# AE-HYU/monte_carlo_localization

Hardware: AMD Instinct MI355X
Metric: MCL updates/sec (particle*beam/s) (higher is better)
Workload: dtype f64; 1 GPU; 4194304 particles/GPU x 1081 beams, Spielberg_map (2000x2000 @ 0.05796), initial cloud N((0.0, 0.0, 0.0),(0.5 m,0.5 m,0.4 rad)) (tracking regime), action (0.05, 0.0, 0.01), stock sensor/motion params, multinomial resampling, Philox seed 42; the timed updates follow 5 warm-up updates (the particle set has resampled to motion-noise width); particles_total=4194304, beams=1081, parallelism=single GPU

## Files before the change

include/mcl_hip_engine.h:

```cpp
#ifndef MCL_HIP_ENGINE_H
#define MCL_HIP_ENGINE_H

#include <stddef.h>
#include <stdint.h>

#ifdef __cplusplus
extern "C" {
#endif

#define MCL_ABI_VERSION 1

typedef struct mcl_engine mcl_engine_t;

typedef enum {
    MCL_OK = 0,
    MCL_ERR_INVALID_ARG = -1,
    MCL_ERR_NOT_READY = -2,
    MCL_ERR_HIP = -3,
    MCL_ERR_NO_DEVICE = -4,
    MCL_ERR_UNSUPPORTED = -5,
    MCL_ERR_PEER = -6,
    MCL_ERR_TIMEOUT = -7
} mcl_status;

// ... 48 lines not shown

int mcl_set_map(mcl_engine_t *h, const int8_t *data, uint32_t width, uint32_t height,
                float resolution, double origin_x, double origin_y);
int mcl_get_max_range_px(const mcl_engine_t *h, int32_t *out);
int mcl_get_sensor_table(const mcl_engine_t *h, double *out, size_t n);

int mcl_set_beam_angles(mcl_engine_t *h, const float *angles, int32_t n_beams);

int mcl_set_particles(mcl_engine_t *h, const double *xyz_colmajor, const double *weights, int64_t n);
int mcl_set_particles_shard(mcl_engine_t *h, const double *xyz_colmajor, const double *weights, int64_t n, double max_weight_of_the_whole_set);
int mcl_init_particles_pose(mcl_engine_t *h, const double pose[3], int64_t n, int64_t first_global_index, int64_t n_total);
int mcl_init_global(mcl_engine_t *h, int64_t n, int64_t first_global_index, int64_t n_total);
int mcl_get_particles(mcl_engine_t *h, double *xyz_colmajor, int64_t n);
int mcl_get_weights(mcl_engine_t *h, double *weights, int64_t n);
int mcl_sample_particles(mcl_engine_t *h, int32_t k, const double *uniforms, double *out_colmajor);
int mcl_particle_mean(mcl_engine_t *h, double out[3]);

int mcl_update(mcl_engine_t *h, const double action[3], const float *obs, int32_t n_beams,
               const double *normals_nx3, const double *uniforms_n);
int mcl_update_scan(mcl_engine_t *h, const double action[3], const float *ranges, int32_t n_ranges, int32_t angle_step);
int mcl_sensor_update(mcl_engine_t *h, const float *obs, int32_t n_beams);

int mcl_expected_pose(mcl_engine_t *h, double out[3]);

int mcl_get_stage_timings(const mcl_engine_t *h, double ms[6]);

int mcl_get_resample_indices(mcl_engine_t *h, int32_t *idx, int64_t n);
int mcl_get_ray_steps(mcl_engine_t *h, uint8_t *steps, size_t n);
int mcl_get_ray_steps16(mcl_engine_t *h, uint16_t *steps, size_t n);
int mcl_get_log_weights(mcl_engine_t *h, double *logw, int64_t n);
int mcl_get_counters(mcl_engine_t *h, uint64_t out[4]);
int mcl_get_compact_list(const mcl_engine_t *h, int64_t *n_entries, int32_t *used_by_last_update);
int mcl_set_debug_count_probes(mcl_engine_t *h, int32_t on);
int mcl_get_ray_kernel_ms(const mcl_engine_t *h, double *ms);
int mcl_get_ray_kernel_id(const mcl_engine_t *h, int32_t *kernel);
int mcl_get_ray_kernel_variant(const mcl_engine_t *h, int32_t out[3]);
int mcl_get_planned_ray_kernel(const mcl_engine_t *h, int64_t n_particles, int32_t *kernel, const char **reason);
int mcl_get_effective_sample_size(const mcl_engine_t *h, double *n_eff, int32_t *resampled_last_update);

typedef struct {
    int64_t min_particles, max_particles;
    double err;
    double z;
    double bin_x_m, bin_y_m;
    int32_t n_theta_bins;
    int32_t round_to;
    int32_t shrink_permille;
    int32_t reserved;
} mcl_kld_config_t;
void mcl_default_kld_config(mcl_kld_config_t *k);
int mcl_set_kld(mcl_engine_t *h, const mcl_kld_config_t *k);
int mcl_get_particle_count(const mcl_engine_t *h, int64_t *n);
int mcl_get_kld_state(const mcl_engine_t *h, int64_t *bins_last, int64_t *n_next);
int mcl_host_kld_bins(const double *x, const double *y, const double *th, int64_t n, uint32_t width, uint32_t height,
                      float resolution, double origin_x, double origin_y, const mcl_kld_config_t *k, int64_t *bins);
int mcl_host_kld_target(const mcl_kld_config_t *k, int64_t bins, int64_t n_current, int64_t *n_next);

typedef struct {
    double bin_x_m, bin_y_m;
    int32_t n_theta_bins;
    int32_t reserved;
} mcl_cluster_config_t;
typedef struct {
    uint64_t weight_q;
    double weight;
    int64_t n_particles, n_bins, first_bin;
// ... 299 lines not shown
```

monte_carlo_localization_amd/csrc/mcl_engine.hip:

```cpp
#include "../../include/mcl_hip_engine.h"

#include <hip/hip_runtime.h>
#include <hip/hip_ext.h>
#include <rocprim/device/device_radix_sort.hpp>

#include <algorithm>
#include <chrono>
#include <cmath>
#include <cstdio>
#include <cstring>
#include <string>
#include <vector>

#include "mcl_engine_internal.h"
#include "mcl_kernels.h"
#include "mcl_host_math.h"
#include "mcl_lfield.h"

static_assert(MCL_WEDGES == mcl::kWedges || MCL_KWEDGES != 16, "include/mcl_hip_engine.h and csrc/mcl_wedge.h disagree");

using namespace mcl_host;

namespace {

// ... 159 lines not shown
void launch_layout(mcl_engine *h, hipStream_t stream, int64_t n, int *bbox, int *tilemark, int *tilemap)
{
    const auto [ntx_abs, nty_abs, tiles_ok] = sort_tiles(h);
    const int bstride = n >= (1 << 20) ? 16 : 1;
    hipLaunchKernelGGL(mcl::k_cell_bbox, dim3((unsigned)std::min<int64_t>((n / bstride + 255) / 256, 128)), dim3(256), 0, stream, h->d_pc, n,
                       bstride, h->Wp, h->Hp, bbox, tiles_ok ? tilemark : (int *)nullptr, ntx_abs);
    if (tiles_ok) hipLaunchKernelGGL(mcl::k_tile_compact, dim3(1), dim3(1024), 0, stream, bbox, tilemark, tilemap, ntx_abs * nty_abs);
}

int launch_far_windowed(mcl_engine *h, const mcl::RayArgs &a, int64_t n, bool count)
{
    const unsigned nb = (unsigned)((n + mcl::kFarTile - 1) / mcl::kFarTile);
    const uint32_t *flags32 = reinterpret_cast<const uint32_t *>(h->d_far.p);
    hipLaunchKernelGGL(mcl::k_far_count, dim3(nb), dim3(256), 0, h->stream, flags32, n, a.far_count, h->d_far_cnt);
    hipLaunchKernelGGL(mcl::k_far_spine, dim3(1), dim3(1024), 0, h->stream, h->d_far_cnt, (int)nb, a.far_count);
    hipLaunchKernelGGL(mcl::k_far_scatter, dim3(nb), dim3(256), 0, h->stream, flags32, n, a.far_count, h->d_far_cnt, h->d_far_sorted);
    const size_t lds = (size_t)h->tw_cells * h->tw_cells / 2;
    if (count) hipLaunchKernelGGL((mcl::k_rays_skip<1, true, true>), dim3(h->num_cu), dim3(mcl::kRayThreads), lds, h->stream, a);
    else hipLaunchKernelGGL((mcl::k_rays_skip<1, false, true>), dim3(h->num_cu), dim3(mcl::kRayThreads), lds, h->stream, a);
    HIPCHK(h, hipGetLastError());
    return MCL_OK;
}

struct RayPlan {
    int mode = 0;
    bool lists = false, ordered = false, sweep = false;
    bool count = false;
    bool timed = false;
    int R = 1;
    int grid = 1;
    size_t lds = 0;
    int nsl = 1, items_per_slice = 4, sweep_g = 1;
    int nseg = 1, fix_split = 1;
    unsigned long long segcap = 0;
    unsigned gfar = 1;
    bool hyb = false, glob = false, rec = false, pairs = false;
    size_t qlds = 0;
    bool far_windowed = false, radix = false;
    bool constants_ready = false, stale_layout = false, keys_written = false, clear_folded = false, obs_wait = false;
    bool heading_form = false;
    mcl::PrepClear clear_passed{};
};

void plan_work_lists(const mcl_engine *h, int64_t n, RayPlan &p)
{
    const int spc = h->env.qslices_per_cu > 0 ? h->env.qslices_per_cu : 32;
    p.nsl = (int)std::max<int64_t>(1, std::min<int64_t>((int64_t)spc * h->num_cu, (n + 255) / 256));
    if (p.ordered) {
        int64_t slice_len = h->env.cell_slice > 0 ? std::max<int64_t>(64, h->env.cell_slice) : (n >= (1 << 21) ? 4096 : 2048);
        p.nsl = (int)std::max<int64_t>(1, (n + slice_len - 1) / slice_len);
    }
    if (p.sweep) {
        p.sweep_g = h->env.sweep_g > 0 ? h->env.sweep_g : 1;
        if (p.sweep_g > mcl::kWedges || (mcl::kWedges % p.sweep_g) != 0) p.sweep_g = 1;
        p.nsl = (int)((n + mcl::kSwUnit - 1) / mcl::kSwUnit);
    }
    p.items_per_slice = p.sweep ? mcl::kWedges / p.sweep_g : (p.ordered ? mcl::kWedges : 4);
    const int max_wg = 2 * (h->num_cu - h->reserved_cus);
    p.nseg = (int)std::min<int64_t>(max_wg, p.items_per_slice * (int64_t)p.nsl);
    const unsigned long long rays_per_seg = (unsigned long long)n * h->B / p.nseg + 64, seg_div = 256;
    p.segcap = std::max<unsigned long long>(2048, (rays_per_seg / seg_div + 7) & ~7ull);
    unsigned long long share = 2;
    if (p.sweep && h->B > 0) {
        const unsigned long long rays = std::max<unsigned long long>(1, (unsigned long long)n * h->B);
        const unsigned long long by_scan = ((unsigned long long)h->wedge_beams_max * p.items_per_slice + h->B - 1) / h->B;
        share = std::max<unsigned long long>(2, std::min<unsigned long long>(by_scan, (8ull << 20) / rays));
    }
    if ((unsigned long long)n * h->B <= (4ull << 20)) p.segcap = (share * rays_per_seg + 7) & ~7ull;
    p.gfar = (unsigned)std::max<int64_t>(1, std::min<int64_t>(4 * (int64_t)h->num_cu, (n + 15) / 16));
    p.fix_split = std::max(1, std::min(16, (8 * h->num_cu) / std::max(p.nseg, 1)));
}

void plan_sweep_form(mcl_engine *h, RayPlan &p)
{
    p.hyb = sweep_hybrid_decide(h);
    p.glob = h->sweep_global && !p.hyb;
    p.rec = h->rec_ok && h->sweep_rec_layout_ok && h->d_beam_err != nullptr && (size_t)mcl::kSwWinBytes + (size_t)h->ltd_cols * 8 <= 80 * 1024 - 64;
    p.far_windowed = sweep_far_expected(h);
    p.pairs = p.rec && !p.hyb && (h->env.sweep_pairs >= 0 ? h->env.sweep_pairs != 0 : (p.glob || p.far_windowed));
    p.qlds = (p.glob ? 0 : (size_t)mcl::kSwWinBytes) + (p.rec ? (size_t)h->ltd_cols * 8 : 0);
}

RayPlan plan_rays(mcl_engine *h, int64_t n, bool force_skip, bool direct_table)
{
    RayPlan p;
    p.mode = choose_ray_mode(h, n, force_skip);
    p.lists = mode_work_lists(p.mode); p.ordered = mode_orders(p.mode); p.sweep = mode_sweep(p.mode);
    p.count = h->cfg.debug_count_probes != 0;
    p.R = h->cfg.rays_per_lane > 0 ? h->cfg.rays_per_lane : 1;
    p.grid = (int)std::max<int64_t>(1, std::min<int64_t>(h->num_cu, (n + 15) / 16));
    p.lds = (size_t)h->tw_cells * h->tw_cells / 2;
    p.timed = !p.lists && !h->capturing && !direct_table;
    const RayHandoff &ho = h->handoff;
    p.constants_ready = ho.constants;
    p.heading_form = ho.heading && ho.keys && ho.stale_layout && mode_sweep(p.mode) && sort_radix(h, n);
    if (ho.heading && !p.heading_form) p.constants_ready = false;
    if (!p.lists) return p;
    plan_work_lists(h, n, p);
    if (p.sweep) plan_sweep_form(h, p);
    else p.qlds = (size_t)h->qside * h->qside;
    p.stale_layout = p.ordered && ho.stale_layout;
    p.keys_written = ho.keys; p.clear_folded = ho.folded; p.clear_passed = ho.passed; p.obs_wait = ho.obs_wait;
    p.radix = p.ordered && sort_radix(h, n);
// ... 154 lines not shown
    a.sweep_g = p.sweep_g; a.Ltd = h->d_Ltd; a.ltd_cols = h->ltd_cols;
    a.split16 = h->env.sw_split16 >= 0 ? h->env.sw_split16 : 0;
    a.beam_csx = h->sweep_global ? h->d_beam_csxg : h->d_beam_csx; a.beam_pad = h->beam_pad; a.beam_margin = h->beam_margin;
    a.beam_csi = h->d_beam_csi; a.beam_err = h->d_beam_err; a.rec_k = 2.0 * h->rec_c;
    a.distg = h->d_distg; a.distg_stride = h->distg_stride; a.distg_pitch = h->distg_pitch;
    a.items = h->d_items; a.centres = h->d_centres; a.nitems = 0; a.nitems_ptr = h->d_nitems; a.unit_sums = h->d_unit_sums; a.unit_begin = h->d_unit_begin; a.slot_space = 1;
    MCL_TRY(h->d_far_list.reserve(h, (size_t)h->cap));
    MCL_TRY(h->d_far_sorted.reserve(h, (size_t)h->cap));
    MCL_TRY(h->d_far_cnt.reserve(h, (size_t)h->cap / mcl::kFarTile + 2));
    a.far_sorted = h->d_far_sorted;
    a.far_windowed = p.far_windowed ? 1 : 0;
    a.far_list = h->d_far_list; a.far_count = h->d_result + 15;
    return MCL_OK;
}

template <bool COUNT>
int ray_kernel_lists(mcl_engine *h, const RayPlan &p, const mcl::RayArgs &a)
{
    const dim3 qg((unsigned)p.nseg), b(mcl::kRayThreads);
    if (!p.sweep) HIPCHK(h, hipEventRecord(h->ev[EV_K0], h->stream));
    if (p.hyb) hipExtLaunchKernelGGL((mcl::k_rays_sweep<COUNT, false, true, false, true>), qg, b, p.qlds, h->stream, nullptr, h->ev[EV_K1], 0, a);
    else if (p.glob && p.rec) hipExtLaunchKernelGGL((mcl::k_rays_sweep<COUNT, true, true, true>), qg, b, p.qlds, h->stream, nullptr, h->ev[EV_K1], 0, a);
    else if (p.glob) hipExtLaunchKernelGGL((mcl::k_rays_sweep<COUNT, true>), qg, b, p.qlds, h->stream, nullptr, h->ev[EV_K1], 0, a);
    else if (p.sweep && p.rec && p.pairs) hipExtLaunchKernelGGL((mcl::k_rays_sweep<COUNT, false, true, true>), qg, b, p.qlds, h->stream, nullptr, h->ev[EV_K1], 0, a);
    else if (p.sweep && p.rec) hipExtLaunchKernelGGL((mcl::k_rays_sweep<COUNT, false, true>), qg, b, p.qlds, h->stream, nullptr, h->ev[EV_K1], 0, a);
    else if (p.sweep) hipExtLaunchKernelGGL((mcl::k_rays_sweep<COUNT>), qg, b, p.qlds, h->stream, nullptr, h->ev[EV_K1], 0, a);
#ifdef MCL_LEGACY_RAY_KERNELS
    else if (p.ordered) hipLaunchKernelGGL((mcl::k_rays_cell<COUNT>), qg, b, p.qlds, h->stream, a);
    else hipLaunchKernelGGL((mcl::k_rays_quad<COUNT>), qg, b, p.qlds, h->stream, a);
#endif
    if (!p.sweep) HIPCHK(h, hipEventRecord(h->ev[EV_K1], h->stream));
    if (p.sweep && p.far_windowed) MCL_TRY(launch_far_windowed(h, a, a.n, COUNT));
    hipLaunchKernelGGL((mcl::k_rays_far<COUNT>), dim3(p.gfar), b, 0, h->stream, a);
    hipLaunchKernelGGL((mcl::k_rays_fix<COUNT>), dim3(p.nseg * p.fix_split), dim3(256), 0, h->stream, a);
    hipLaunchKernelGGL((mcl::k_rays_exact<COUNT>), dim3(2 * h->num_cu), dim3(256), 0, h->stream, a);
    return MCL_OK;
}
template int ray_kernel_lists<true>(mcl_engine *, const RayPlan &, const mcl::RayArgs &);
template int ray_kernel_lists<false>(mcl_engine *, const RayPlan &, const mcl::RayArgs &);

int ray_kernel(mcl_engine *h, const RayPlan &p, const mcl::RayArgs &a)
{
    if (p.lists) return p.count ? ray_kernel_lists<true>(h, p, a) : ray_kernel_lists<false>(h, p, a);
    const dim3 g(p.grid), b(mcl::kRayThreads);
    if (p.timed) HIPCHK(h, hipEventRecord(h->ev[EV_K0], h->stream));
    if (p.mode == MCL_RAYS_MARCH) ray_kernel_march(h, p, a);
    else if (p.count) hipLaunchKernelGGL((mcl::k_rays_skip<1, true>), g, b, p.lds, h->stream, a);
    else {
        switch (p.R) {
        case 1: hipLaunchKernelGGL((mcl::k_rays_skip<1, false>), g, b, p.lds, h->stream, a); break;
        case 2: hipLaunchKernelGGL((mcl::k_rays_skip<2, false>), g, b, p.lds, h->stream, a); break;
        case 3: hipLaunchKernelGGL((mcl::k_rays_skip<3, false>), g, b, p.lds, h->stream, a); break;
        default: hipLaunchKernelGGL((mcl::k_rays_skip<4, false>), g, b, p.lds, h->stream, a); break;
        }
    }
    if (p.timed) HIPCHK(h, hipEventRecord(h->ev[EV_K1], h->stream));
    return MCL_OK;
}

void ray_combine(mcl_engine *h, const RayPlan &p, int64_t n)
{
    if (p.sweep) {
        hipExtLaunchKernelGGL(mcl::k_combine_logw, dim3(mcl::kRedBlocks), dim3(256), 0, h->stream, nullptr, h->ev[EV_RAYS], 0, n, h->d_perm.p, h->d_logw_acc.p,
                              h->d_logw.p, h->d_maxpart.p, h->d_fix_count.p, p.nseg, p.segcap, h->d_fix_over);
        h->stage_ev.rays_bound = true;
        h->max_partials_ready = true;
    } else {
// ... 363 lines not shown
    h->h_fix_count = h->h_result[12];
    uint64_t qt;
    std::memcpy(&qt, &h->h_scalars[2], 8);
    h->q_total = qt;
    h->global_sums[0] = h->h_scalars[1];
    h->global_sums[1] = h->h_scalars[3];
    h->global_sums[2] = h->h_scalars[4];
    h->global_sums[3] = h->h_scalars[5];
    h->global_sums[4] = h->h_scalars[6];
    if (h->compact_pending) {
        const unsigned long long na = h->h_result[16];
        h->compact_n = na <= (unsigned long long)h->compact_cap ? (int64_t)na : -1;
        h->compact_pending = false;
    }
}

int mcl_abi_version(void) { return MCL_ABI_VERSION; }

const char *mcl_last_error(const mcl_engine_t *h) { return h ? h->err.c_str() : g_create_error.c_str(); }

static EnvKnobs read_knobs()
{
    EnvKnobs k;
    if (const char *e = getenv("MCL_CELL_MIN")) k.cell_min = atoll(e);
    if (const char *e = getenv("MCL_CELL_SLICE")) k.cell_slice = atoll(e);
    if (const char *e = getenv("MCL_QSLICES_PER_CU")) k.qslices_per_cu = atoi(e);
    if (const char *e = getenv("MCL_QSIDE")) k.qside = atoi(e);
    if (const char *e = getenv("MCL_SWEEP_G")) k.sweep_g = atoi(e);
    if (const char *e = getenv("MCL_TINY_POLL")) k.tiny_poll = atoi(e);
    if (const char *e = getenv("MCL_NO_COMPACT")) k.no_compact = atoi(e);
    if (const char *e = getenv("MCL_SORT")) k.sort_radix = std::strcmp(e, "radix") == 0 ? 1 : (std::strcmp(e, "hist") == 0 ? 0 : -1);
    if (const char *e = getenv("MCL_SORT_FINE")) k.sort_fine = atoi(e);
    if (const char *e = getenv("MCL_SORT_FINE_SUB")) k.sort_fine_sub = atoi(e);
    if (const char *e = getenv("MCL_DEBUG_WG")) k.debug_wg = e;
    k.no_bucket_cuts = getenv("MCL_NO_BUCKET_CUTS") != nullptr;
    if (const char *e = getenv("MCL_SWEEP_GLOBAL")) k.sweep_global = atoi(e) != 0;
    if (const char *e = getenv("MCL_SWEEP_HYBRID")) k.sweep_hybrid = atoi(e);
    if (const char *e = getenv("MCL_SW_GUIDE")) k.sw_guide = atoi(e);
    if (const char *e = getenv("MCL_SW_SPLIT16")) k.sw_split16 = atoi(e) != 0;
    if (const char *e = getenv("MCL_SWEEP_PAIRS")) k.sweep_pairs = atoi(e) != 0 ? 1 : 0;
    k.no_obs_overlap = getenv("MCL_NO_OBS_OVERLAP") != nullptr;
    k.no_prep_fold = getenv("MCL_NO_PREP_FOLD") != nullptr;
    k.no_stale_layout = getenv("MCL_NO_STALE_LAYOUT") != nullptr;
    k.comm_no_pregather = getenv("MCL_COMM_NO_PREGATHER") != nullptr;
    k.comm_no_lists = getenv("MCL_COMM_NO_LISTS") != nullptr;
    return k;
}

int mcl_create(const mcl_config_t *cfg, mcl_engine_t **out)
{
    if (cfg && (cfg->resample_neff_permille < 0 || cfg->resample_neff_permille > 1000)) return MCL_ERR_INVALID_ARG;
    g_create_error.clear();
    if (!cfg || !out) { g_create_error = "null argument"; return MCL_ERR_INVALID_ARG; }
    *out = nullptr;
    if (cfg->max_particles <= 0 || cfg->max_particles >= MCL_MAX_TOTAL_PARTICLES || cfg->squash_factor <= 0 || cfg->max_range_m <= 0) {
        g_create_error = "bad config (max_particles must be in [1, 2^27) / squash_factor / max_range_m)";
        return MCL_ERR_INVALID_ARG;
    }
    if (!std::isfinite(cfg->squash_factor) || !std::isfinite(cfg->max_range_m)) {
        g_create_error = "bad config (squash_factor and max_range_m must be finite)";
        return MCL_ERR_INVALID_ARG;
    }
    if (const char *why = bad_sensor_fields(*cfg)) { g_create_error = why; return MCL_ERR_INVALID_ARG; }
    {
        const double disp[3] = {cfg->motion_dispersion_x, cfg->motion_dispersion_y, cfg->motion_dispersion_theta};
        for (double v : disp)
// ... 1079 lines not shown
{
    if (!h || !logw) return MCL_ERR_INVALID_ARG;
    if (!h->have_logw) return MCL_ERR_NOT_READY;
    if (n != h->N) return MCL_ERR_INVALID_ARG;
    HIPCHK(h, hipSetDevice(h->cfg.device));
    HIPCHK(h, hipMemcpyAsync(logw, h->d_logw, (size_t)n * 8, hipMemcpyDeviceToHost, h->stream));
    HIPCHK(h, hipStreamSynchronize(h->stream));
    return MCL_OK;
}

int mcl_get_counters(mcl_engine_t *h, uint64_t out[4])
{
    if (!h || !out) return MCL_ERR_INVALID_ARG;
    for (int i = 0; i < 4; ++i) out[i] = h->h_counters[i];
    return MCL_OK;
}

int mcl_get_compact_list(const mcl_engine_t *h, int64_t *n_entries, int32_t *used_by_last_update)
{
    if (!h || !n_entries || !used_by_last_update) return MCL_ERR_INVALID_ARG;
    *n_entries = h->compact_n;
    *used_by_last_update = h->compact_used ? 1 : 0;
    return MCL_OK;
}

int mcl_set_debug_count_probes(mcl_engine_t *h, int32_t on)
{
    if (!h) return MCL_ERR_INVALID_ARG;
    graph_reset(h);
    h->cfg.debug_count_probes = on ? 1 : 0;
    return MCL_OK;
}

int mcl_get_ray_kernel_ms(const mcl_engine_t *h, double *ms)
{
    if (!h || !ms) return MCL_ERR_INVALID_ARG;
    *ms = h->ray_ms;
    return MCL_OK;
}

int mcl_get_ray_kernel_id(const mcl_engine_t *h, int32_t *kernel)
{
    if (!h || !kernel) return MCL_ERR_INVALID_ARG;
    if (const int rc = lf_refuse_rays(h)) return rc;
    *kernel = h->last_mode;
    return MCL_OK;
}

int mcl_get_ray_kernel_variant(const mcl_engine_t *h, int32_t out[3])
{
    if (!h || !out) return MCL_ERR_INVALID_ARG;
    if (const int rc = lf_refuse_rays(h)) return rc;
    out[0] = h->last_sweep_global; out[1] = h->last_sweep_rec; out[2] = h->last_sweep_pairs;
    return MCL_OK;
}

int mcl_get_planned_ray_kernel(const mcl_engine_t *h, int64_t n_particles, int32_t *kernel, const char **reason)
{
    if (!h || !kernel) return MCL_ERR_INVALID_ARG;
    if (!h->have_map || h->B <= 0) return MCL_ERR_NOT_READY;
    const int64_t n = n_particles > 0 ? n_particles : (h->have_particles ? h->N : h->cap);
    const char *why = "";
    *kernel = choose_ray_mode(h, n, false, &why);
    if (reason) *reason = why ? why : "";
    return MCL_OK;
}
// ... 928 lines not shown
```

monte_carlo_localization_amd/csrc/mcl_engine_internal.h:

```cpp
#pragma once
#include "../../include/mcl_hip_engine.h"

#include <hip/hip_runtime.h>
#include <hip/hip_ext.h>

#include <cstdint>
#include <string>
#include <vector>

#include "mcl_types.h"
#include "mcl_host_math.h"
#include "mcl_buffers.h"

enum { EV_START = 0, EV_RESAMPLE, EV_QUERY, EV_RAYS, EV_SENSOR, EV_K0, EV_K1, EV_COUNT };


constexpr unsigned long long kExactCap = 1ull << 16;
constexpr int kResultWords = 18;
constexpr int kResultStage = 40;
constexpr int kResultStamp = 32;

struct mcl_comm;
void comm_free(struct mcl_comm *c);
void comm_forget(struct mcl_comm *c);
struct mcl_cluster;
void cluster_free(struct mcl_cluster *c);
struct mcl_query;
void query_free(struct mcl_query *q);
struct mcl_search;
void search_free(struct mcl_search *s);
struct mcl_refine;
void refine_free(struct mcl_refine *r);

struct RayHandoff {
    bool constants = false;
    bool stale_layout = false;
    bool keys = false;
    bool heading = false;
    bool folded = false; mcl::PrepClear passed{};
    bool obs_wait = false;
};
struct StageEvents {
    bool rays_bound = false;
    bool query_skipped = false;
};
struct NextLayout {
    bool wanted = false, pending = false, valid = false; int64_t n = 0;
    hipEvent_t ev_children = nullptr, ev_layout = nullptr;
    DevBuf<int> d_bbox_nx, d_tilemap_nx, d_tilemark_nx;
};
struct EnvKnobs {
    int64_t cell_min = 0, cell_slice = 0;
    int qslices_per_cu = 0, qside = 0, sweep_g = 0;
    int tiny_poll = 1, no_compact = 0;
    int sort_radix = -1;
    int sort_fine = -1;
    int sort_fine_sub = -1;
    std::string debug_wg;
    bool no_bucket_cuts = false;
    bool sweep_global = false;
    int sweep_hybrid = 1;
    int sw_guide = 0;
    int sw_split16 = -1;
    int sweep_pairs = -1;
    bool no_obs_overlap = false;
    bool no_prep_fold = false;
    bool no_stale_layout = false;
    bool comm_no_pregather = false;
    bool comm_no_lists = false;
};

struct OrderLast { const int *bbox = nullptr, *tilemap = nullptr; int64_t n = 0; int fine = 0; bool heading = false; };

struct mcl_engine {
    mcl_config_t cfg{};
    int num_cu = 256;
    hipStream_t stream = nullptr;
    hipStream_t stream2 = nullptr;
    std::string err;
    bool have_map = false;
    int W = 0, H = 0, P = 0, Wp = 0, Hp = 0, Wps = 0, tw_cells = 0;
    double res = 0, ox = 0, oy = 0;
    std::vector<double> table;
    DevBuf<int8_t> d_grid;
    DevBuf<uint8_t> d_dist;
    DevBuf<uint8_t> d_dist4;
    DevBuf<uint8_t> d_distq[4];
    DevBuf<uint8_t> d_distw;
    DevBuf<float> d_L;
    DevBuf<double> d_table;
// ... 240 lines not shown
```

monte_carlo_localization_amd/csrc/mcl_kernels.h:

```cpp
#pragma once
#include "mcl_types.h"
#include <type_traits>
#include "mcl_ray_core.h"
#include "mcl_device_math.h"
#include "mcl_wedge.h"
#include "mcl_motion.h"
#include "mcl_sort_key.h"

namespace mcl {

constexpr int kRedBlocks = 1024;
constexpr int kRedThreads = 256;
__device__ __forceinline__ void final_sums_of(const double *__restrict__ part, int nb, double *__restrict__ scalars, double (*sm)[7]);


__device__ __forceinline__ uint64_t wave_incl_scan_u64(uint64_t v, int lane)
{
#pragma unroll
    for (int o = 1; o < 64; o <<= 1) {
        uint64_t t = (uint64_t)__shfl_up((long long)v, o, 64);
        if (lane >= o) v += t;
    }
    return v;
}
// ... 1378 lines not shown
        sy = sm[0][1] + sm[1][1] + sm[2][1] + sm[3][1];
        cnt = sm[0][2] + sm[1][2] + sm[2][2] + sm[3][2];
        out[blockIdx.x] = cnt > 0.0 ? make_double2(sx / cnt, sy / cnt) : make_double2(0.0, 0.0);
    }
}

template <bool GRID = false>
__device__ __forceinline__ int first_beam_in_wedge(double th, const float *__restrict__ angle, int B, int m, double a0, double inv_inc)
{
    int lo = 0, hi = B;
    const double x = ((double)m * (6.283185307179586476925286766559 / kWedges) - th - a0) * inv_inc;
    if (x > -4.0 && x < (double)B + 4.0) {
        const int jg = min(max((int)ceil(x), 0), B);
        if (GRID && fabs(x - rint(x)) > 4e-6 * inv_inc + 1e-6) return jg;
        const bool below = jg == 0 || beam_wedge(th, angle[jg - 1]) < m;
        const bool at = jg == B || beam_wedge(th, angle[jg]) >= m;
        if (below && at) return jg;
        const int l = max(jg - 2, 0), h = min(jg + 2, B);
        if ((l == 0 || beam_wedge(th, angle[l - 1]) < m) && (h == B || beam_wedge(th, angle[h]) >= m)) { lo = l; hi = h; }
    }
    while (lo < hi) {
        const int mid = (lo + hi) >> 1;
        if (beam_wedge(th, angle[mid]) >= m) hi = mid; else lo = mid + 1;
    }
    return lo;
}

#ifdef MCL_LEGACY_RAY_KERNELS
}
#include "mcl_rays_legacy.h"
namespace mcl {
#endif

template <bool COUNT>
__global__ __launch_bounds__(256) void k_rays_fix(RayArgs a)
{
    unsigned long long cnt_exact = 0, cnt_probe = 0, cnt_l2 = 0;
    const int split = max(1, (int)gridDim.x / a.fix_segments);
    const int part = blockIdx.x % split;
    for (int seg = blockIdx.x / split; seg < a.fix_segments; seg += gridDim.x / split) {
    unsigned long long n = 0;
    if (threadIdx.x == 0) n = a.slot_space ? a.fix_count[(size_t)seg * 8] : atomicAdd(&a.fix_count[(size_t)seg * 8], 0ull);
    n = __shfl((long long)n, 0, 64);
    {
        __shared__ unsigned long long n_sh;
        if (threadIdx.x == 0) n_sh = n;
        __syncthreads();
        n = n_sh;
        __syncthreads();
    }
    if (n > a.fix_cap) n = 0;
    cnt_l2 += (threadIdx.x == 0 && part == 0) ? n : 0;
    const unsigned long long *list = a.fix_list + (size_t)seg * a.fix_cap;
    for (unsigned long long k = (unsigned long long)part * blockDim.x + threadIdx.x; k < n; k += (unsigned long long)blockDim.x * split) {
        const unsigned long long e = a.slot_space ? list[k] : atomicAdd(const_cast<unsigned long long *>(&list[k]), 0ull);
        const int64_t p = (int64_t)(e >> 16);
        const int j = (int)(e & 0xFFFF);
        const double4 pci = a.slot_space ? a.pcs[p] : a.pc[p];
        const uint8_t *wfield = nullptr;
        if (a.slot_space && a.distw) {
            const double hth = a.ths[p];
            if (hth == hth && fabs(hth) < 1e6) wfield = a.distw + (size_t)(beam_wedge(hth, a.beam_angle[j]) & (kWedges - 1)) * a.distw_stride;
        }
        const double2 cs = a.beam_cs[j];
        const double ux = pci.x * cs.x - pci.y * cs.y, uy = pci.y * cs.x + pci.x * cs.y;
        const RayOrigin o = ray_origin(a, pci.z, pci.w);
        int r = a.P;
        uint32_t amb = o.amb0;
        unsigned np = 0;
        if (o.sane)
            r = trace_fp64<false, COUNT>(a, nullptr, 0, kOriginBase, o.p0x, o.p0y, ux, uy, first_skip(a, o, wfield ? wfield : a.dist, wfield != nullptr),
                                         amb, np, wfield, wfield != nullptr);
        if (takes_literal_march(a, o.sane, amb)) {
            if (a.exact_list) {
                const unsigned long long slot = atomicAdd(a.exact_count, 1ull);
                if (slot < a.exact_cap) { atomicExch(&a.exact_list[slot], e); continue; }
            }
            const int64_t i = a.slot_space ? (int64_t)a.perm[p] : p;
            r = march_exact(a, a.x[i], a.y[i], a.th[i] + (double)a.beam_angle[j]);
            ++cnt_exact;
        }
        atomicAdd(&a.logw[p], (double)a.Lt[(size_t)r * a.bpad + j]);
        if (a.steps || a.steps16) store_step(a, a.slot_space ? (int64_t)a.perm[p] : p, j, r);
        if (COUNT) cnt_probe += np;
    }
    }
    if (a.counters) {
        if (cnt_exact) atomicAdd(&a.counters[0], cnt_exact);
        if (COUNT && cnt_probe) atomicAdd(&a.counters[2], cnt_probe);
        if (cnt_l2) atomicAdd(&a.counters[3], cnt_l2);
    }
}

template <bool COUNT>
__global__ __launch_bounds__(256) void k_rays_exact(RayArgs a)
{
    const int lane = threadIdx.x & 63;
    const unsigned long long wave_id = ((unsigned long long)blockIdx.x * blockDim.x + threadIdx.x) >> 6;
    const unsigned long long nwaves = ((unsigned long long)gridDim.x * blockDim.x) >> 6;
    unsigned long long n = 0;
    if (lane == 0) n = atomicAdd(a.exact_count, 0ull);
    n = (unsigned long long)__shfl((long long)n, 0, 64);
    if (n > a.exact_cap) n = a.exact_cap;
    unsigned long long done = 0;
    for (unsigned long long k = wave_id; k < n; k += nwaves) {
        unsigned long long e = 0;
        if (lane == 0) e = atomicAdd(&a.exact_list[k], 0ull);
        e = (unsigned long long)__shfl((long long)e, 0, 64);
        const int64_t p = (int64_t)(e >> 16);
        const int64_t i = a.slot_space ? (int64_t)a.perm[p] : p;
        const int j = (int)(e & 0xFFFF);
        const double angle = a.th[i] + (double)a.beam_angle[j];
        const double dx = cos(angle) * a.res, dy = sin(angle) * a.res;
        const int r = wave_march_exact_dir(a, a.x[i], a.y[i], dx, dy, lane);
        if (lane == 0) {
            atomicAdd(&a.logw[p], (double)a.Lt[(size_t)r * a.bpad + j]);
            if (a.steps || a.steps16) store_step(a, i, j, r);
            ++done;
// ... 490 lines not shown
```

monte_carlo_localization_amd/engine.py:

```python
from __future__ import annotations

import ctypes as C
import os

import numpy as np

_HERE = os.path.dirname(os.path.abspath(__file__))
LIB_PATH = os.environ.get("MCL_LIB") or os.path.join(_HERE, "libmcl_hip_engine.so")

MCL_OK = 0
MCL_ERR_INVALID_ARG = -1
MCL_ERR_NOT_READY = -2
MCL_ERR_PEER = -6
MCL_ERR_TIMEOUT = -7
RESAMPLE_MULTINOMIAL, RESAMPLE_SYSTEMATIC = 0, 1
WEIGHT_LOG, WEIGHT_PRODUCT = 0, 1
RAYS_AUTO, RAYS_MARCH, RAYS_SKIP, RAYS_QUAD, RAYS_CELL, RAYS_SWEEP = 0, 1, 2, 3, 4, 5
BUF_X, BUF_Y, BUF_THETA, BUF_QWEIGHT, BUF_LOGW, BUF_SCALARS = range(6)

EXPORTS = [
    "mcl_abi_version", "mcl_default_config", "mcl_create", "mcl_destroy", "mcl_last_error", "mcl_set_map",
    "mcl_get_max_range_px", "mcl_get_sensor_table", "mcl_set_beam_angles", "mcl_set_particles",
    "mcl_get_particles", "mcl_get_weights", "mcl_sample_particles", "mcl_particle_mean", "mcl_update",
    "mcl_sensor_update", "mcl_expected_pose", "mcl_get_stage_timings", "mcl_get_resample_indices",
    "mcl_get_ray_steps", "mcl_get_log_weights", "mcl_get_counters", "mcl_get_ray_kernel_ms", "mcl_device_ptr",
    "mcl_stage_propagate", "mcl_stage_weights", "mcl_stage_finish", "mcl_scan_weights", "mcl_export_state",
    "mcl_get_scalars", "mcl_host_sensor_table", "mcl_host_skip_field", "mcl_init_particles_pose", "mcl_init_global",
    "mcl_update_scan", "mcl_get_ray_kernel_id", "mcl_host_skip_field_dir", "mcl_host_skip_field_wedge", "mcl_export_records", "mcl_get_effective_sample_size", "mcl_get_host_scalars", "mcl_stage_resample_records", "mcl_stage_resample", "mcl_stage_rays",
    "mcl_set_reserved_cus", "mcl_stage_resample_indices", "mcl_stage_motion_records", "mcl_stage_distinct_parents", "mcl_export_records_at",
    "mcl_group_create", "mcl_group_destroy", "mcl_group_last_error", "mcl_group_size", "mcl_group_engine", "mcl_group_set_map",
    "mcl_group_set_beam_angles", "mcl_group_set_particles", "mcl_group_init_particles_pose", "mcl_group_init_global",
    "mcl_group_update", "mcl_group_expected_pose", "mcl_group_get_particles", "mcl_group_get_weights",
    "mcl_group_get_resample_indices", "mcl_group_get_stage_timings", "mcl_group_exchange_bytes",
    "mcl_set_debug_count_probes", "mcl_set_particles_shard", "mcl_get_compact_list", "mcl_compact_chunk_bytes", "mcl_export_compact",
    "mcl_stage_resample_compact", "mcl_group_exchanged_lists", "mcl_get_ray_steps16", "mcl_get_planned_ray_kernel",
    "mcl_stream_wait_external", "mcl_external_wait_stream", "mcl_export_compact_async", "mcl_stage_resample_compact_async",
    "mcl_stage_rays_async", "mcl_stage_weights_async", "mcl_stage_complete", "mcl_stage_keep",
    "mcl_comm_available", "mcl_comm_unique_id", "mcl_comm_create", "mcl_comm_destroy", "mcl_comm_update", "mcl_comm_stats", "mcl_comm_set_lists", "mcl_comm_get_vector", "mcl_comm_last_exchange", "mcl_comm_selftest",
    "mcl_host_sweep_global_layout", "mcl_get_ray_kernel_variant", "mcl_host_skip_field_wedge_tight", "mcl_host_wedge_tight_table",
    "mcl_get_wedge_fields", "mcl_get_ring_fields", "mcl_get_sweep_table", "mcl_host_sort_key", "mcl_get_sort_order", "mcl_get_sort_record_form",
    "mcl_default_kld_config", "mcl_set_kld", "mcl_get_particle_count", "mcl_get_kld_state", "mcl_host_kld_bins", "mcl_host_kld_target",
    "mcl_default_cluster_config", "mcl_pose_clusters", "mcl_get_cluster_labels",
    "mcl_query_scans", "mcl_score_poses", "mcl_get_query_counters",
    "mcl_default_search_config", "mcl_global_search", "mcl_get_search_scores", "mcl_get_search_bytes", "mcl_host_search_lattice",
    "mcl_host_search_headings", "mcl_init_particles_mixture",
    "mcl_global_search_sequence", "mcl_host_search_sequence_offsets", "mcl_host_relative_poses",
    "mcl_default_search_stream_config", "mcl_global_search_streamed", "mcl_host_search_slabs",
    "mcl_global_search_beam", "mcl_host_search_beam_grid", "mcl_get_search_beam_table",
    "mcl_default_search_prune_config", "mcl_global_search_pruned", "mcl_get_search_bounds", "mcl_host_search_blocks", "mcl_host_lf_pool",
    "mcl_host_search_bound_table", "mcl_host_search_prune_next", "mcl_global_search_sequence_pruned",
    "mcl_default_refine_config", "mcl_refine_poses", "mcl_refine_poses_beam", "mcl_get_refine_scores", "mcl_get_refine_bytes", "mcl_host_refine_window",
    "mcl_host_refine_reduce", "mcl_refine_poses_sequence", "mcl_host_refine_sequence_offsets",
    "mcl_default_recovery_config", "mcl_set_recovery", "mcl_get_recovery_state", "mcl_set_recovery_state", "mcl_host_recovery_step",
    "mcl_set_recovery_proposal", "mcl_get_recovery_proposal", "mcl_host_recovery_proposal",
    "mcl_default_likelihood_field_config", "mcl_set_likelihood_field", "mcl_get_likelihood_field", "mcl_get_likelihood_table",
    "mcl_host_likelihood_field", "mcl_host_likelihood_table",
    "mcl_default_beam_skip_config", "mcl_set_beam_skip", "mcl_get_beam_skip_state", "mcl_host_beam_skip_thresholds",
    "mcl_host_beam_skip_plan",
    "mcl_default_motion_config", "mcl_set_motion_model", "mcl_get_motion_model", "mcl_host_motion_scalars", "mcl_host_motion_sample",
    "mcl_init_particles_gaussian", "mcl_host_gaussian_factor", "mcl_group_set_motion_model", "mcl_group_init_particles_gaussian",
]
MOTION_REFERENCE, MOTION_DIFF, MOTION_OMNI = 0, 1, 2
MOTION_MODELS = {"reference": MOTION_REFERENCE, "diff": MOTION_DIFF, "omni": MOTION_OMNI}


class Config(C.Structure):
    _fields_ = [
# ... 1399 lines not shown
    def resample_indices(self):
        out = np.empty(self.n, np.int32)
        self._chk(self.lib.mcl_get_resample_indices(self._h, _p(out), C.c_int64(self.n)), "mcl_get_resample_indices")
        return out

    def ray_steps(self):
        if self.max_range_px > 255:
            out = np.empty(self.n * self.n_beams, np.uint16)
            self._chk(self.lib.mcl_get_ray_steps16(self._h, _p(out), C.c_size_t(out.size)), "mcl_get_ray_steps16")
        else:
            out = np.empty(self.n * self.n_beams, np.uint8)
            self._chk(self.lib.mcl_get_ray_steps(self._h, _p(out), C.c_size_t(out.size)), "mcl_get_ray_steps")
        return out.reshape(self.n, self.n_beams)

    def log_weights(self):
        out = np.empty(self.n, np.float64)
        self._chk(self.lib.mcl_get_log_weights(self._h, _p(out), C.c_int64(self.n)), "mcl_get_log_weights")
        return out

    def counters(self):
        out = np.zeros(4, np.uint64)
        self._chk(self.lib.mcl_get_counters(self._h, _p(out)), "mcl_get_counters")
        return dict(exact_fallback_rays=int(out[0]), off_window_particles=int(out[1]), probes=int(out[2]),
                    level2_rays=int(out[3]))

    def compact_list(self):
        n, u = C.c_int64(), C.c_int32()
        self._chk(self.lib.mcl_get_compact_list(self._h, C.byref(n), C.byref(u)), "mcl_get_compact_list")
        return n.value, bool(u.value)

    def set_debug_count_probes(self, on):
        self._chk(self.lib.mcl_set_debug_count_probes(self._h, C.c_int32(1 if on else 0)), "mcl_set_debug_count_probes")

    def ray_kernel_ms(self):
        v = C.c_double()
        self._chk(self.lib.mcl_get_ray_kernel_ms(self._h, C.byref(v)), "mcl_get_ray_kernel_ms")
        return v.value

    def effective_sample_size(self):
        v, r = C.c_double(), C.c_int32()
        self._chk(self.lib.mcl_get_effective_sample_size(self._h, C.byref(v), C.byref(r)), "mcl_get_effective_sample_size")
        return v.value, bool(r.value)

    def ray_kernel_name(self):
        v = C.c_int32()
        self._chk(self.lib.mcl_get_ray_kernel_id(self._h, C.byref(v)), "mcl_get_ray_kernel_id")
        return {1: "k_rays_march", 2: "k_rays_skip", 3: "k_rays_quad", 4: "k_rays_cell", 5: "k_rays_sweep"}.get(v.value, "?")

    def ray_kernel_variant(self):
        v = (C.c_int32 * 3)()
        self._chk(self.lib.mcl_get_ray_kernel_variant(self._h, v), "mcl_get_ray_kernel_variant")
        return dict(global_fields=v[0] == 1, hybrid=v[0] == 2, turned_directions=bool(v[1]), pairs=bool(v[2]))

    RAY_KERNEL_NAMES = {0: None, 1: "k_rays_march", 2: "k_rays_skip", 3: "k_rays_quad", 4: "k_rays_cell", 5: "k_rays_sweep"}

    def planned_ray_kernel(self, n_particles=0):
        v, why = C.c_int32(), C.c_char_p()
        self._chk(self.lib.mcl_get_planned_ray_kernel(self._h, C.c_int64(int(n_particles)), C.byref(v), C.byref(why)), "mcl_get_planned_ray_kernel")
        return self.RAY_KERNEL_NAMES.get(v.value, "?"), (why.value or b"").decode()

    def device_ptr(self, which) -> int:
        p = C.c_void_p()
        self._chk(self.lib.mcl_device_ptr(self._h, C.c_int32(which), C.byref(p)), "mcl_device_ptr")
        return int(p.value or 0)

    def export_state(self, d_x=0, d_y=0, d_th=0, d_q=0):
# ... 302 lines not shown
```

Baseline: 924.9 billion particle*beam/s.

## Flatten fix-ray work across segments and merge per-wave logw atomics

```diff
diff --git a/include/mcl_hip_engine.h b/include/mcl_hip_engine.h
--- a/include/mcl_hip_engine.h
+++ b/include/mcl_hip_engine.h
@@ -104,6 +104,7 @@
 int mcl_get_counters(mcl_engine_t *h, uint64_t out[4]);
 int mcl_get_compact_list(const mcl_engine_t *h, int64_t *n_entries, int32_t *used_by_last_update);
 int mcl_set_debug_count_probes(mcl_engine_t *h, int32_t on);
+int mcl_set_debug_force_exact(mcl_engine_t *h, int32_t level);
 int mcl_get_ray_kernel_ms(const mcl_engine_t *h, double *ms);
 int mcl_get_ray_kernel_id(const mcl_engine_t *h, int32_t *kernel);
 int mcl_get_ray_kernel_variant(const mcl_engine_t *h, int32_t out[3]);
diff --git a/monte_carlo_localization_amd/csrc/mcl_engine.hip b/monte_carlo_localization_amd/csrc/mcl_engine.hip
--- a/monte_carlo_localization_amd/csrc/mcl_engine.hip
+++ b/monte_carlo_localization_amd/csrc/mcl_engine.hip
@@ -215,6 +215,7 @@
     size_t lds = 0;
     int nsl = 1, items_per_slice = 4, sweep_g = 1;
     int nseg = 1, fix_split = 1;
+    bool fix_flat = false; int fix_grid = 1;
     unsigned long long segcap = 0;
     unsigned gfar = 1;
     bool hyb = false, glob = false, rec = false, pairs = false;
@@ -251,7 +252,9 @@
     }
     if ((unsigned long long)n * h->B <= (4ull << 20)) p.segcap = (share * rays_per_seg + 7) & ~7ull;
     p.gfar = (unsigned)std::max<int64_t>(1, std::min<int64_t>(4 * (int64_t)h->num_cu, (n + 15) / 16));
-    p.fix_split = std::max(1, std::min(16, (8 * h->num_cu) / std::max(p.nseg, 1)));
+    p.fix_split = std::max(1, std::min(16, (mcl::kFixWgPerCu * h->num_cu) / std::max(p.nseg, 1)));
+    p.fix_flat = !h->env.fix_deal_seg && p.nseg <= mcl::kFixSegMax && (unsigned long long)p.nseg * p.segcap < (1ull << 32);
+    p.fix_grid = p.fix_flat ? std::max(1, (h->env.fix_wg > 0 ? std::min(h->env.fix_wg, 16) : mcl::kFixWgPerCu) * h->num_cu) : p.nseg * p.fix_split;
 }
 
 void plan_sweep_form(mcl_engine *h, RayPlan &p)
@@ -472,7 +475,7 @@
     if (!p.sweep) HIPCHK(h, hipEventRecord(h->ev[EV_K1], h->stream));
     if (p.sweep && p.far_windowed) MCL_TRY(launch_far_windowed(h, a, a.n, COUNT));
     hipLaunchKernelGGL((mcl::k_rays_far<COUNT>), dim3(p.gfar), b, 0, h->stream, a);
-    hipLaunchKernelGGL((mcl::k_rays_fix<COUNT>), dim3(p.nseg * p.fix_split), dim3(256), 0, h->stream, a);
+    hipLaunchKernelGGL((mcl::k_rays_fix<COUNT>), dim3((unsigned)p.fix_grid), dim3(256), 0, h->stream, a, p.fix_flat ? 1 : 0);
     hipLaunchKernelGGL((mcl::k_rays_exact<COUNT>), dim3(2 * h->num_cu), dim3(256), 0, h->stream, a);
     return MCL_OK;
 }
@@ -902,6 +905,8 @@
     if (const char *e = getenv("MCL_SORT")) k.sort_radix = std::strcmp(e, "radix") == 0 ? 1 : (std::strcmp(e, "hist") == 0 ? 0 : -1);
     if (const char *e = getenv("MCL_SORT_FINE")) k.sort_fine = atoi(e);
     if (const char *e = getenv("MCL_SORT_FINE_SUB")) k.sort_fine_sub = atoi(e);
+    if (const char *e = getenv("MCL_FIX_WG")) k.fix_wg = atoi(e);
+    if (const char *e = getenv("MCL_FIX_DEAL")) k.fix_deal_seg = std::strcmp(e, "seg") == 0;
     if (const char *e = getenv("MCL_DEBUG_WG")) k.debug_wg = e;
     k.no_bucket_cuts = getenv("MCL_NO_BUCKET_CUTS") != nullptr;
     if (const char *e = getenv("MCL_SWEEP_GLOBAL")) k.sweep_global = atoi(e) != 0;
@@ -2047,6 +2052,14 @@
     return MCL_OK;
 }
 
+int mcl_set_debug_force_exact(mcl_engine_t *h, int32_t level)
+{
+    if (!h || level < 0 || level > 2) return MCL_ERR_INVALID_ARG;
+    graph_reset(h);
+    h->cfg.debug_force_exact = level;
+    return MCL_OK;
+}
+
 int mcl_get_ray_kernel_ms(const mcl_engine_t *h, double *ms)
 {
     if (!h || !ms) return MCL_ERR_INVALID_ARG;
diff --git a/monte_carlo_localization_amd/csrc/mcl_engine_internal.h b/monte_carlo_localization_amd/csrc/mcl_engine_internal.h
--- a/monte_carlo_localization_amd/csrc/mcl_engine_internal.h
+++ b/monte_carlo_localization_amd/csrc/mcl_engine_internal.h
@@ -56,6 +56,8 @@
     int sort_radix = -1;
     int sort_fine = -1;
     int sort_fine_sub = -1;
+    int fix_wg = 0;
+    bool fix_deal_seg = false;
     std::string debug_wg;
     bool no_bucket_cuts = false;
     bool sweep_global = false;
diff --git a/monte_carlo_localization_amd/csrc/mcl_kernels.h b/monte_carlo_localization_amd/csrc/mcl_kernels.h
--- a/monte_carlo_localization_amd/csrc/mcl_kernels.h
+++ b/monte_carlo_localization_amd/csrc/mcl_kernels.h
@@ -1434,30 +1434,35 @@
 namespace mcl {
 #endif
 
+constexpr int kFixSegMax = 1024;
+constexpr int kFixWgPerCu = 6;
+
+__device__ __forceinline__ void wave_run_add(double *__restrict__ acc, int64_t p, bool add, double v, int lane)
+{
+    const long long key = add ? (long long)p : -1ll;
+    const long long prev = __shfl_up(key, 1, 64);
+    const bool head = lane == 0 || !add || prev != key;
+    const unsigned long long heads = __ballot(head);
+    const unsigned long long above = lane == 63 ? 0ull : heads >> (lane + 1);
+    const int next = above ? lane + __ffsll((long long)above) : 64;
+#pragma unroll
+    for (int d = 1; d < 64; d <<= 1) {
+        const double o = __shfl_down(v, d, 64);
+        if (lane + d < next) v += o;
+    }
+    if (head && add) atomicAdd(&acc[p], v);
+}
+
 template <bool COUNT>
-__global__ __launch_bounds__(256) void k_rays_fix(RayArgs a)
-{
-    unsigned long long cnt_exact = 0, cnt_probe = 0, cnt_l2 = 0;
-    const int split = max(1, (int)gridDim.x / a.fix_segments);
-    const int part = blockIdx.x % split;
-    for (int seg = blockIdx.x / split; seg < a.fix_segments; seg += gridDim.x / split) {
-    unsigned long long n = 0;
-    if (threadIdx.x == 0) n = a.slot_space ? a.fix_count[(size_t)seg * 8] : atomicAdd(&a.fix_count[(size_t)seg * 8], 0ull);
-    n = __shfl((long long)n, 0, 64);
-    {
-        __shared__ unsigned long long n_sh;
-        if (threadIdx.x == 0) n_sh = n;
-        __syncthreads();
-        n = n_sh;
-        __syncthreads();
-    }
-    if (n > a.fix_cap) n = 0;
-    cnt_l2 += (threadIdx.x == 0 && part == 0) ? n : 0;
-    const unsigned long long *list = a.fix_list + (size_t)seg * a.fix_cap;
-    for (unsigned long long k = (unsigned long long)part * blockDim.x + threadIdx.x; k < n; k += (unsigned long long)blockDim.x * split) {
-        const unsigned long long e = a.slot_space ? list[k] : atomicAdd(const_cast<unsigned long long *>(&list[k]), 0ull);
-        const int64_t p = (int64_t)(e >> 16);
-        const int j = (int)(e & 0xFFFF);
+__device__ __forceinline__ void fix_ray(const RayArgs &a, unsigned long long e, bool valid, int lane, unsigned long long &cnt_exact,
+                                        unsigned long long &cnt_probe)
+{
+    const int64_t p = (int64_t)(e >> 16);
+    const int j = (int)(e & 0xFFFF);
+    bool add = valid;
+    int r = a.P;
+    unsigned np = 0;
+    if (valid) {
         const double4 pci = a.slot_space ? a.pcs[p] : a.pc[p];
         const uint8_t *wfield = nullptr;
         if (a.slot_space && a.distw) {
@@ -1467,25 +1472,104 @@
         const double2 cs = a.beam_cs[j];
         const double ux = pci.x * cs.x - pci.y * cs.y, uy = pci.y * cs.x + pci.x * cs.y;
         const RayOrigin o = ray_origin(a, pci.z, pci.w);
-        int r = a.P;
         uint32_t amb = o.amb0;
-        unsigned np = 0;
         if (o.sane)
             r = trace_fp64<false, COUNT>(a, nullptr, 0, kOriginBase, o.p0x, o.p0y, ux, uy, first_skip(a, o, wfield ? wfield : a.dist, wfield != nullptr),
                                          amb, np, wfield, wfield != nullptr);
         if (takes_literal_march(a, o.sane, amb)) {
+            bool handed = false;
             if (a.exact_list) {
                 const unsigned long long slot = atomicAdd(a.exact_count, 1ull);
-                if (slot < a.exact_cap) { atomicExch(&a.exact_list[slot], e); continue; }
+                if (slot < a.exact_cap) { atomicExch(&a.exact_list[slot], e); handed = true; }
             }
-            const int64_t i = a.slot_space ? (int64_t)a.perm[p] : p;
-            r = march_exact(a, a.x[i], a.y[i], a.th[i] + (double)a.beam_angle[j]);
-            ++cnt_exact;
-        }
-        atomicAdd(&a.logw[p], (double)a.Lt[(size_t)r * a.bpad + j]);
+            if (!handed) {
+                const int64_t i = a.slot_space ? (int64_t)a.perm[p] : p;
+                r = march_exact(a, a.x[i], a.y[i], a.th[i] + (double)a.beam_angle[j]);
+                ++cnt_exact;
+            }
+            add = !handed;
+        }
+    }
+    const double v = add ? (double)a.Lt[(size_t)r * a.bpad + j] : 0.0;
+    wave_run_add(a.logw, p, add, v, lane);
+    if (add) {
         if (a.steps || a.steps16) store_step(a, a.slot_space ? (int64_t)a.perm[p] : p, j, r);
         if (COUNT) cnt_probe += np;
     }
+}
+
+template <bool COUNT>
+__global__ __launch_bounds__(256) void k_rays_fix(RayArgs a, int flat)
+{
+    __shared__ uint32_t pre[kFixSegMax + 1];
+    __shared__ uint32_t wsum[4];
+    __shared__ unsigned long long n_sh;
+    unsigned long long cnt_exact = 0, cnt_probe = 0, cnt_l2 = 0;
+    const int lane = threadIdx.x & 63;
+    if (flat) {
+        const int nseg = a.fix_segments;
+        uint32_t c[4], t = 0;
+#pragma unroll
+        for (int i = 0; i < 4; ++i) {
+            const int seg = (int)threadIdx.x * 4 + i;
+            unsigned long long n = 0;
+            if (seg < nseg) n = a.slot_space ? a.fix_count[(size_t)seg * 8] : atomicAdd(&a.fix_count[(size_t)seg * 8], 0ull);
+            if (n > a.fix_cap) n = 0;
+            c[i] = (uint32_t)n;
+            t += c[i];
+        }
+        uint32_t inc = t;
+#pragma unroll
+        for (int d = 1; d < 64; d <<= 1) {
+            const uint32_t up = __shfl_up(inc, d, 64);
+            if (lane >= d) inc += up;
+        }
+        if (lane == 63) wsum[threadIdx.x >> 6] = inc;
+        __syncthreads();
+        uint32_t run = inc - t;
+        for (int w = 0; w < (int)(threadIdx.x >> 6); ++w) run += wsum[w];
+        if (threadIdx.x == 0) pre[0] = 0;
+#pragma unroll
+        for (int i = 0; i < 4; ++i) {
+            const int seg = (int)threadIdx.x * 4 + i;
+            run += c[i];
+            if (seg < nseg) pre[seg + 1] = run;
+        }
+        __syncthreads();
+        const unsigned long long total = pre[nseg];
+        if (blockIdx.x == 0 && threadIdx.x == 0) cnt_l2 = total;
+        for (unsigned long long base = (unsigned long long)blockIdx.x * 256; base < total; base += (unsigned long long)gridDim.x * 256) {
+            const unsigned long long idx = base + threadIdx.x;
+            const bool valid = idx < total;
+            const uint32_t ic = (uint32_t)(valid ? idx : total - 1);
+            int lo = 0, hi = nseg - 1;
+            for (int it = 0; it < 11 && lo < hi; ++it) {
+                const int mid = (lo + hi) >> 1;
+                if (pre[mid + 1] <= ic) lo = mid + 1; else hi = mid;
+            }
+            const unsigned long long *src = a.fix_list + (size_t)lo * a.fix_cap + (ic - pre[lo]);
+            const unsigned long long e = a.slot_space ? *src : atomicAdd(const_cast<unsigned long long *>(src), 0ull);
+            fix_ray<COUNT>(a, e, valid, lane, cnt_exact, cnt_probe);
+        }
+    } else {
+        const int split = max(1, (int)gridDim.x / a.fix_segments);
+        const int part = blockIdx.x % split;
+        for (int seg = blockIdx.x / split; seg < a.fix_segments; seg += gridDim.x / split) {
+            if (threadIdx.x == 0) n_sh = a.slot_space ? a.fix_count[(size_t)seg * 8] : atomicAdd(&a.fix_count[(size_t)seg * 8], 0ull);
+            __syncthreads();
+            unsigned long long n = n_sh;
+            __syncthreads();
+            if (n > a.fix_cap) n = 0;
+            cnt_l2 += (threadIdx.x == 0 && part == 0) ? n : 0;
+            const unsigned long long *list = a.fix_list + (size_t)seg * a.fix_cap;
+            for (unsigned long long base = (unsigned long long)part * 256; base < n; base += (unsigned long long)split * 256) {
+                const unsigned long long idx = base + threadIdx.x;
+                const bool valid = idx < n;
+                const unsigned long long ic = valid ? idx : n - 1;
+                const unsigned long long e = a.slot_space ? list[ic] : atomicAdd(const_cast<unsigned long long *>(&list[ic]), 0ull);
+                fix_ray<COUNT>(a, e, valid, lane, cnt_exact, cnt_probe);
+            }
+        }
     }
     if (a.counters) {
         if (cnt_exact) atomicAdd(&a.counters[0], cnt_exact);
diff --git a/monte_carlo_localization_amd/engine.py b/monte_carlo_localization_amd/engine.py
--- a/monte_carlo_localization_amd/engine.py
+++ b/monte_carlo_localization_amd/engine.py
@@ -32,7 +32,7 @@
     "mcl_group_set_beam_angles", "mcl_group_set_particles", "mcl_group_init_particles_pose", "mcl_group_init_global",
     "mcl_group_update", "mcl_group_expected_pose", "mcl_group_get_particles", "mcl_group_get_weights",
     "mcl_group_get_resample_indices", "mcl_group_get_stage_timings", "mcl_group_exchange_bytes",
-    "mcl_set_debug_count_probes", "mcl_set_particles_shard", "mcl_get_compact_list", "mcl_compact_chunk_bytes", "mcl_export_compact",
+    "mcl_set_debug_count_probes", "mcl_set_debug_force_exact", "mcl_set_particles_shard", "mcl_get_compact_list", "mcl_compact_chunk_bytes", "mcl_export_compact",
     "mcl_stage_resample_compact", "mcl_group_exchanged_lists", "mcl_get_ray_steps16", "mcl_get_planned_ray_kernel",
     "mcl_stream_wait_external", "mcl_external_wait_stream", "mcl_export_compact_async", "mcl_stage_resample_compact_async",
     "mcl_stage_rays_async", "mcl_stage_weights_async", "mcl_stage_complete", "mcl_stage_keep",
@@ -1498,6 +1498,9 @@
     def set_debug_count_probes(self, on):
         self._chk(self.lib.mcl_set_debug_count_probes(self._h, C.c_int32(1 if on else 0)), "mcl_set_debug_count_probes")
 
+    def set_debug_force_exact(self, level):
+        self._chk(self.lib.mcl_set_debug_force_exact(self._h, C.c_int32(int(level))), "mcl_set_debug_force_exact")
+
     def ray_kernel_ms(self):
         v = C.c_double()
         self._chk(self.lib.mcl_get_ray_kernel_ms(self._h, C.byref(v)), "mcl_get_ray_kernel_ms")
```

Result: faster. 938.3 billion particle*beam/s, median of 6 (+1.5%).
